# Plachtaa/FAcodec

Measured on AMD Instinct MI355X. Metric: 24kHz audio sec encoded+decoded per wall-sec, higher is better.
Workload: dtype f32; 1 GPU; configs[1]: batch=32/GPU x 2 s @ 24 kHz, forward encoder->FVQ(6 codebooks)->decoder, FAcodec configs/config.yml model (137.7 M params), weights formula-generated, weight-norm re-materialised every step; clips_per_gpu=32, samples_per_clip=48000, parallelism=dp1 (independent clips, no collective)

## Files before the change

### facodec_amd/_lib.py

```python
import ctypes as C
import os

_HERE = os.path.dirname(os.path.abspath(__file__))
LIB_PATH = os.environ.get("FAC_LIB_PATH", os.path.join(_HERE, "libfacodec_hip.so"))

PAD_ZERO, PAD_REFLECT = 0, 1
ACT_NONE, ACT_TANH, ACT_MISH, ACT_LOG_MEL = 0, 1, 2, 3
ACT_GATE, ACT_WN_RES_SKIP = 4, 5

_p = C.c_void_p
_i = C.c_int
_i64 = C.c_int64
_f = C.c_float


class ConvDesc(C.Structure):
    _fields_ = [
        ("x", _p), ("w", _p), ("bias", _p), ("alpha_in", _p), ("alpha_out", _p), ("res", _p), ("y", _p), ("y2", _p), ("alpha_y2", _p), ("w_k1", _p), ("bias_k1", _p),
        ("x_bs", _i64), ("x_cs", _i64), ("y_bs", _i64), ("y_cs", _i64),
        ("B", C.c_int32), ("C_in", C.c_int32), ("T_in", C.c_int32), ("C_out", C.c_int32),
        ("C_out_pad", C.c_int32), ("T_out", C.c_int32),
        ("K", C.c_int32), ("stride", C.c_int32), ("dilation", C.c_int32), ("pad_left", C.c_int32),
        ("pad_mode", C.c_int32), ("n_phase", C.c_int32), ("y_tstride", C.c_int32), ("phase_shift", C.c_int32),
        ("act", C.c_int32),
        ("w_batched", C.c_int32), ("w_bs", _i64), ("ws", _p), ("ws_bytes", _i64), ("w_split", _p),
        ("K1", C.c_int32), ("dilation2", C.c_int32), ("row_phases", C.c_int32),
        ("x_p8", _p), ("x_p8_plane_bytes", _i64), ("y2_p8", _p), ("y2_p8_plane_bytes", _i64),
        ("pw_split", C.c_int32), ("split_rows", C.c_int32),
        ("gate_cond", _p), ("gate_cond_bs", _i64),
    ]


class VqDesc(C.Structure):
    _fields_ = [
        ("residual", _p), ("z_in", _p), ("zq_acc", _p), ("zq_out", _p), ("w_in", _p), ("b_in", _p),
        ("codebook", _p), ("w_out", _p), ("w_out_scale", _p), ("b_out", _p), ("mask", _p), ("codes", _p), ("z_e", _p),
        ("loss_part", _p), ("codes_bs", _i64),
        ("B", C.c_int32), ("D", C.c_int32), ("T", C.c_int32), ("Kc", C.c_int32),
    ]



VQ_DECODE_MAX_Q = 16


class VqDecodeDesc(C.Structure):
    _fields_ = [
        ("codes", _p * 3), ("codes_bs", _i64 * 3), ("codes_qs", _i64 * 3), ("n_q", C.c_int32 * 3),
        ("codebook", _p * VQ_DECODE_MAX_Q), ("w_out", _p * VQ_DECODE_MAX_Q), ("w_out_scale", _p * VQ_DECODE_MAX_Q),
        ("b_out", _p * VQ_DECODE_MAX_Q), ("style", _p), ("outs", _p), ("z", _p * 3),
        ("B", C.c_int32), ("D", C.c_int32), ("T", C.c_int32), ("Kc", C.c_int32),
    ]


class CodesPackDesc(C.Structure):
    _fields_ = [
        ("codes", _p * 3), ("codes_bs", _i64 * 3), ("codes_qs", _i64 * 3), ("n_q", C.c_int32 * 3),
        ("lens", _p), ("out", _p), ("out_bs", _i64),
        ("B", C.c_int32), ("T", C.c_int32), ("bits", C.c_int32),
    ]


# ... 147 lines not shown
    "fac_spec_to_cat": (_i, [_p, _p, _i, _i, _i, _i, _i, _i, _i, _p]),
    "fac_period_fold": (_i, [_p, _p, _i, _i, _i, _i, _i, _i, _p]),
    "fac_zero_insert": (_i, [_p, _p, _i64, _i, _i, _p]),
    "fac_row_stack3": (_i, [_p, _p, _i64, _i, _i, _i, _i, _p]),
    "fac_spec_to_rows": (_i, [_p, _p, _i, _i, _i, _i, _i, _i, _p]),
    "fac_pad_reflect": (_i, [_p, _p, _i, _i, _i, _i, _p]),
    "fac_disc_preprocess": (_i, [_p, _p, _p, _p, _i, _i, _p]),
    "fac_cross_entropy": (_i, [_p, _p, _p, _p, _p, _i64, _i, _f, _p]),
    "fac_focal_scalar": (_i, [_p, _p, _f, _p]),
    "fac_crop_rows": (_i, [_p, _p, _p, _i, _i, _i64, _i, _i, _p]),
    "fac_stream_push": (_i, [_p, _p, _i64, _i64, _i, _i, _i, _p]),
    "fac_vq_fwd": (_i, [C.POINTER(VqDesc), _p]),
    "fac_vq_loss_tiles": (_i, [_i]),
    "fac_vq_decode": (_i, [C.POINTER(VqDecodeDesc), _p]),
    "fac_codes_pack": (_i, [C.POINTER(CodesPackDesc), _p]),
    "fac_codes_unpack": (_i, [C.POINTER(CodesUnpackDesc), _p]),
    "fac_codes_row_bytes": (_i64, [_i, _i, _i]),
    "fac_rccl_available": (_i, []),
    "fac_rccl_unique_id": (_i, [_p]),
    "fac_rccl_comm_init": (_i, [C.POINTER(_p), _p, _i, _i]),
    "fac_rccl_comm_destroy": (_i, [_p]),
    "fac_allreduce_arena": (_i, [_p, _p, _i64, _i, _p]),
    "fac_vq_search": (_i, [_p, _p, _p, _i64, _i, _p]),
    "fac_gate_tanh_sigmoid": (_i, [_p, _p, _i64, _p, _i, _i, _i, _p]),
    "fac_embed_sum": (_i, [_p, _p, _p, _i, _i, _i, _i, _i, _i, _i, _i, _p]),
    "fac_glu_residual": (_i, [_p, _p, _p, _i, _i, _i, _p]),
    "fac_add": (_i, [_p, _p, _p, _i64, _p]),
    "fac_sub2": (_i, [_p, _p, _p, _p, _i64, _p]),
    "fac_mul_mask": (_i, [_p, _p, _i, _i, _i, _p]),
    "fac_wn_res_skip": (_i, [_p, _p, _p, _i, _i, _i, _i, _p]),
    "fac_attention": (_i, [_p, _p, _p, _p, _p, _i, _i, _i, _i, _p]),
    "fac_attention_stream": (_i, [_p, _p, _p, _p, _p, _i, _i, _i, _i, _p]),
    "fac_attention_route": (_i, [_i, _i]),
    "fac_attention_stream_tile": (_i, [_i]),
    "fac_masked_mean": (_i, [_p, _p, _p, _i, _i, _i, _p]),
    "fac_layernorm_c_affine": (_i, [_p, _p, _p, _i, _i, _i, _p]),
    "fac_stft_frames": (_i, [_p, _p, _i, _i, _i, _i, _i, _i, _i, _p]),
    "fac_stft_frames_ragged": (_i, [_p, _p, _p, _i, _i, _i, _i, _i, _i, _i, _p]),
    "fac_mask_tail": (_i, [_p, _p, _i, _i, _i, _i, _p]),
    "fac_mask_tail_i64": (_i, [_p, _p, _i, _i, _i, _i, _p]),
    "fac_edge_tail": (_i, [_p, _p, _i, _i, _i, _i, _i, _i, _p]),
    "fac_frame_mask": (_i, [_p, _p, _p, _i, _i, _i, _p]),
    "fac_resample": (_i, [C.POINTER(ResampleDesc), _p]),
    "fac_resample_form": (_i, [C.POINTER(ResampleDesc), _p]),
    "fac_kweight_ws_bytes": (_i64, [_i, _i]),
    "fac_kweight_energy": (_i, [C.POINTER(KweightDesc), _p]),
    "fac_loudness_chunk": (_i, [_i]),
    "fac_loudness_gate": (_i, [_p, _i64, _p, _i64, _i, _i, _p, _i, _p, _p, _i, _p]),
    "fac_loudness_gain": (_i, [_p, _i64, _p, _p, _p, _p, C.c_double, _i, _p, _i64, _p, _i, _i, _p]),
    "fac_si_sdr_ws_bytes": (_i64, [_i, _i]),
    "fac_si_sdr": (_i, [_p, _i64, _p, _i64, _p, _p, _p, _i64, _i, _i, _p]),
    "fac_stoi_geometry": (_i, [_i, C.POINTER(_i64)]),
    "fac_stoi_select": (_i, [C.POINTER(StoiDesc), _p]),
    "fac_stoi_bands": (_i, [C.POINTER(StoiDesc), _p]),
    "fac_stoi_score": (_i, [C.POINTER(StoiDesc), _p]),
    "fac_slot_copy": (_i, [_p, _i, _p, _i, _i, _i, C.POINTER(C.c_int32), _i, _p]),
    "fac_rows_pick": (_i, [_p, _i64, _p, _p, _i, _i, _i, _p]),
    "fac_spec_power": (_i, [_p, _p, _i, _i, _i, _i, _p]),
    "fac_reduce_pair": (_i, [_p, _p, _p, _p, _i64, _i, _f, _f, _i, _p]),
    "fac_aa_snakebeta_fwd": (_i, [_p, _p, _p, _p, _p, _i, _i, _i, _p]),
    "fac_logdiff_rms": (_i, [_p, _p, _p, _p, _i, _i, _i, _f, _f, _i, _p]),
    "fac_jdc_affine_lrelu_pool": (_i, [_p, _p, _p, _p, _i, _i, _i, _i, _i, _i, _i, _f, _p]),
    "fac_jdc_layout_in": (_i, [_p, _p, _i, _i, _i, _i, _p]),
    "fac_jdc_to_time_major": (_i, [_p, _p, _i, _i, _i, _i, _i, _i, _i, _p]),
    "fac_jdc_to_nchw": (_i, [_p, _p, _i, _i, _i, _i, _i, _i, _p]),
    "fac_jdc_head": (_i, [_p, _p, _p, _p, _p, _i, _i, _i, _i, _p]),
# ... 34 lines not shown
```

### facodec_amd/build.py

```python
import os
import subprocess
import sys
from concurrent.futures import ThreadPoolExecutor

HERE = os.path.dirname(os.path.abspath(__file__))
CSRC = os.path.join(HERE, "csrc")
TAG = os.environ.get("FAC_BUILD_TAG", "")
LIB = os.path.join(HERE, "libfacodec_hip%s.so" % ("_" + TAG if TAG else ""))
OBJDIR = "build" + ("_" + TAG if TAG else "")
SOURCES = ["conv1d_api.hip", "conv1d_tile_128x128.hip", "conv1d_tile_96x128.hip", "conv1d_tile_64x128.hip",
           "conv1d_tile_32x256.hip", "conv1d_tile_128x32.hip", "conv1d_tile_128x256.hip", "conv1d_fused_ru.hip", "conv1d_narrow.hip", "conv1d_pw.hip", "conv1d_pw_split.hip", "conv1d_skinny.hip", "conv1d_bsplit.hip", "conv1d_bsplit96.hip", "conv1d_gemm_split.hip", "conv1d_bsplit2.hip", "conv1d_bwd.hip", "conv1d_wgrad_split.hip", "conv1d_wgrad_k1.hip", "train_misc.hip", "optim.hip", "train_quant.hip", "train_pred.hip", "train_disc.hip", "train_redecoder.hip", "pack.hip", "prep_batch.hip", "lstm.hip", "lstm_persist.hip", "vq.hip", "vq_decode.hip", "bitpack.hip", "misc.hip", "attention_stream.hip", "ragged.hip", "resample.hip", "loudness.hip", "metrics.hip", "stream_pool.hip", "jdc.hip", "rccl_arena.hip"]
FLAGS = ["--offload-arch=gfx950", "-O3", "-std=c++17", "-fPIC", "-ffp-contract=off",
         "-Wno-unused-result"] + os.environ.get("FAC_EXTRA_FLAGS", "").split()


def _hipcc():
    for cand in (os.environ.get("HIPCC"), "/opt/rocm/bin/hipcc", "hipcc"):
        if cand and (os.path.isabs(cand) and os.path.exists(cand) or not os.path.isabs(cand)):
            return cand
    return "hipcc"


def _stale(target, deps):
    if not os.path.exists(target):
        return True
    tt = os.path.getmtime(target)
    return any(os.path.getmtime(d) > tt for d in deps)


def build_lib(force=False, verbose=True):
    hipcc = _hipcc()
    headers = sorted(os.path.join(CSRC, f) for f in os.listdir(CSRC) if f.endswith(".h")) + [os.path.join(HERE, "..", "include", "facodec_hip.h")]
    objs, jobs = [], []
    os.makedirs(os.path.join(CSRC, OBJDIR), exist_ok=True)
    for src in SOURCES:
        s = os.path.join(CSRC, src)
        o = os.path.join(CSRC, OBJDIR, src.replace(".hip", ".o"))
        objs.append(o)
        if force or _stale(o, [s] + headers):
            jobs.append([hipcc, *FLAGS, "-c", s, "-o", o])

    def run(cmd):
        if verbose:
            print(" ".join(cmd), file=sys.stderr)
# ... 13 lines not shown
```

### facodec_amd/csrc/conv1d_api.hip

```cpp
#include "conv1d_mfma.h"
#include <stdlib.h>

namespace fac {

enum ConvKernel : int {
  CK_128x32 = 0,
  CK_32x256 = 1,
  CK_64x128 = 2,
  CK_96x128 = 3,
  CK_128x128 = 4,
  CK_128x256 = 5,
  CK_96x256 = 6,
  CK_FUSED_RU = 7,
  CK_128x160 = 8,
  CK_NARROW = 9,
  CK_SKINNY = 10,
  CK_BSPLIT = 11,
  CK_CIN1 = 12,
  CK_THIN = 13,
  CK_PW = 14,
  CK_GSPLIT = 15,
  CK_BSPLIT2 = 16,
  CK_PWS = 17,
  CK_PWT = 18,
  CK_BSPLIT96 = 19,
};

static ConvKernel select_variant(const fac_conv_desc* d) {
  const int co = d->C_out;
  if (d->row_phases > 1) return CK_128x256;
  if (d->T_out <= 32) return CK_128x32;
  if (co <= 32) return CK_32x256;
  if (co <= 64) return CK_64x128;
  const bool wide = d->K == 1 && d->n_phase == 1 && d->T_out >= 512;
  if (d->T_out > 128 && d->T_out <= 160 && co > 64) return CK_128x160;
  if (co % 128 != 0 && co % 96 == 0) return wide ? CK_96x256 : CK_96x128;
  return wide ? CK_128x256 : CK_128x128;
}

static bool narrow_ok(const fac_conv_desc* d) {
  return d->C_out <= 2 && d->stride == 1 && d->n_phase == 1 && d->phase_shift == 0 && d->y_tstride == 1 && !d->res && !d->y2 &&
         !d->w_batched && d->y && (long long)d->B <= 65535 && (long long)d->B * ((d->T_out + 1023) / 1024) >= 128;
}

static bool pw_enabled() {
  static const bool on = !(getenv("FAC_PW") && getenv("FAC_PW")[0] == '0');
  return on;
}

static int conv_plan(const fac_conv_desc* d, ConvArgs& a, ConvKernel& k) {
  FAC_REQUIRE(d && (d->x || d->x_p8) && (d->w || d->w_split) && (d->y || d->y2 || d->y2_p8), "conv1d: null pointer");
  FAC_REQUIRE(!d->y2 || d->alpha_y2 || d->act == FAC_ACT_WN_RES_SKIP, "conv1d: y2 needs alpha_y2");
  FAC_REQUIRE(d->B > 0 && d->C_in > 0 && d->C_out > 0 && d->T_in > 0 && d->T_out > 0,
              "conv1d: bad shape B=%d C_in=%d C_out=%d T_in=%d T_out=%d", d->B, d->C_in, d->C_out,
              d->T_in, d->T_out);
  FAC_REQUIRE(d->K >= 1 && d->stride >= 1 && d->dilation >= 1 && d->pad_left >= 0,
              "conv1d: bad K/stride/dilation/pad");
  FAC_REQUIRE(d->C_out_pad % 32 == 0 && (d->C_out_pad >= d->C_out || d->row_phases > 1), "conv1d: C_out_pad must be a multiple of 32");
  FAC_REQUIRE(d->n_phase >= 1 && d->y_tstride >= 1, "conv1d: bad phase config");
  FAC_REQUIRE((long long)d->B * d->n_phase <= 65535, "conv1d: B*n_phase too large for grid.z");
  a.x = d->x; a.w = d->w; a.bias = d->bias; a.alpha_in = d->alpha_in; a.alpha_out = d->alpha_out;
  a.res = d->res; a.y = d->y; a.y2 = d->y2; a.alpha2 = d->alpha_y2;
  a.w1 = d->w_k1; a.bias1 = d->bias_k1;
  a.x_p8 = reinterpret_cast<const unsigned char*>(d->x_p8); a.x_p8_ps = d->x_p8_plane_bytes;
  a.y2_p8 = reinterpret_cast<unsigned char*>(d->y2_p8); a.y2_p8_ps = d->y2_p8_plane_bytes;
  FAC_REQUIRE(!d->y2_p8 || d->alpha_y2, "conv1d: y2_p8 needs alpha_y2");
  if (d->w_k1) {
    FAC_REQUIRE(d->C_in == d->C_out && d->C_out_pad == d->C_out && d->n_phase == 1 && d->stride == 1 &&
// ... 168 lines not shown
```

### facodec_amd/csrc/misc.hip

```cpp
#include "common.h"
#include <string.h>

namespace fac {

static thread_local char g_err[512] = "";

void set_error(const char* fmt, ...) {
  va_list ap;
  va_start(ap, fmt);
  vsnprintf(g_err, sizeof(g_err), fmt, ap);
  va_end(ap);
}

constexpr int EW_THREADS = 256;
inline int ew_grid(long long n, int per_thread = 1) {
  long long g = (n + (long long)EW_THREADS * per_thread - 1) / ((long long)EW_THREADS * per_thread);
  if (g > 8192) g = 8192;
  if (g < 1) g = 1;
  return (int)g;
}

__global__ void snake_kernel(const float* __restrict__ x, const float* __restrict__ alpha,
                             float* __restrict__ y, int C, int T, long long n) {
  for (long long i = (long long)blockIdx.x * blockDim.x + threadIdx.x; i < n;
// ... 537 lines not shown
  if (threadIdx.x == 0) scratch[blockIdx.x] = (part[0] + part[1]) + (part[2] + part[3]);
}

__global__ __launch_bounds__(256) void logdiff_rms_bwd_kernel(const float* __restrict__ a, const float* __restrict__ b,
                                                              float* __restrict__ db, int M, int T, long long n_cols, float eps,
                                                              float scale, int accumulate) {
  for (long long i = (long long)blockIdx.x * 256 + threadIdx.x; i < n_cols; i += (long long)gridDim.x * 256) {
    const long long bb = i / T;
    const int t = (int)(i - bb * T);
    const float* pa = a + bb * M * T + t;
    const float* pb = b + bb * M * T + t;
    float* pd = db + bb * M * T + t;
    float q = 0.f;
    for (int m = 0; m < M; ++m) {
      const float d = logf(fabsf(pa[(long long)m * T]) + eps) - logf(fabsf(pb[(long long)m * T]) + eps);
      q = fmaf(d, d, q);
    }
    const float r = sqrtf(q / (float)M);
    const float k = r > 0.f ? scale / ((float)M * r) : 0.f;
    for (int m = 0; m < M; ++m) {
      const float bv = pb[(long long)m * T];
      const float d = logf(fabsf(pa[(long long)m * T]) + eps) - logf(fabsf(bv) + eps);
      const float sg = bv > 0.f ? 1.f : (bv < 0.f ? -1.f : 0.f);
      const float g = -k * d * sg / (fabsf(bv) + eps);
      pd[(long long)m * T] = accumulate ? pd[(long long)m * T] + g : g;
    }
  }
}

}

using namespace fac;

extern "C" int fac_version(void) { return 4; }
extern "C" const char* fac_last_error(void) { return fac::g_err; }

#define EW_LAUNCH(kern, n, ...)                                                         \
  hipLaunchKernelGGL(kern, dim3(ew_grid(n)), dim3(EW_THREADS), 0, (hipStream_t)stream, __VA_ARGS__)

extern "C" int fac_snake_fwd(const float* x, const float* alpha, float* y, int B, int C, int T,
                             fac_stream_t stream) {
  FAC_REQUIRE(x && alpha && y && B > 0 && C > 0 && T > 0, "snake_fwd: bad arguments");
  const long long n = (long long)B * C * T;
  if (T >= 1024 && (long long)B * C <= 65535) {
    hipLaunchKernelGGL(snake_rows_kernel, dim3((T + 1023) / 1024, B * C), dim3(256), 0, (hipStream_t)stream, x, alpha, y, C, T);
  } else {
    EW_LAUNCH(snake_kernel, n, x, alpha, y, C, T, n);
  }
  return check_launch("snake_fwd");
}

extern "C" int fac_gate_tanh_sigmoid(const float* a, const float* g, int64_t g_bs, float* out, int B,
                                     int C, int T, fac_stream_t stream) {
  FAC_REQUIRE(a && out && B > 0 && C > 0 && T > 0, "gate_tanh_sigmoid: bad arguments");
  const long long n = (long long)B * C * T;
  EW_LAUNCH(gate_kernel, n, a, g, out, C, T, (long long)g_bs, n);
  return check_launch("gate_tanh_sigmoid");
}

extern "C" int fac_embed_sum(const int64_t* codes, const float* tables, float* out, int B, int n_tab,
                             int n_codes, int code_row0, int V, int E, int T, int accumulate,
                             fac_stream_t stream) {
  FAC_REQUIRE(codes && tables && out && B > 0 && n_tab >= 0 && V > 0 && E > 0 && T > 0 &&
                  code_row0 >= 0 && code_row0 + n_tab <= n_codes, "embed_sum: bad arguments");
  const long long n = (long long)B * E * T;
  EW_LAUNCH(embed_sum_kernel, n, (const long long*)codes, tables, out, n_tab, n_codes, code_row0, V, E, T, n,
            accumulate);
// ... 21 lines not shown
  return check_launch("sub2");
}

extern "C" int fac_mul_mask(float* x, const float* mask, int B, int C, int T, fac_stream_t stream) {
  FAC_REQUIRE(x && mask && B > 0 && C > 0 && T > 0, "mul_mask: bad arguments");
  const long long n = (long long)B * C * T;
  EW_LAUNCH(mul_mask_kernel, n, x, mask, C, T, n);
  return check_launch("mul_mask");
}

extern "C" int fac_stream_push(float* buf, const float* src, int64_t rows, int64_t cap, int hist, int n_prev,
                               int n_new, fac_stream_t stream) {
  FAC_REQUIRE(buf && src && rows > 0 && hist >= 0 && hist <= 2048 && n_prev >= 0 && n_new > 0 &&
                  cap >= (int64_t)hist + n_new && cap >= (int64_t)hist + n_prev,
              "stream_push: bad arguments (rows=%lld cap=%lld hist=%d n_prev=%d n_new=%d)", (long long)rows,
              (long long)cap, hist, n_prev, n_new);
  hipLaunchKernelGGL(stream_push_kernel, dim3((unsigned)rows), dim3(256), 0, (hipStream_t)stream, buf, src,
                     (long long)cap, hist, n_prev, n_new);
  return check_launch("stream_push");
}

extern "C" int fac_wn_res_skip(const float* rs, float* x, float* out, int B, int C, int T, int last,
                               fac_stream_t stream) {
  FAC_REQUIRE(rs && out && (last || x) && B > 0 && C > 0 && T > 0, "wn_res_skip: bad arguments");
  const long long n = (long long)B * C * T;
  EW_LAUNCH(wn_res_skip_kernel, n, rs, x, out, C, T, last, n);
  return check_launch("wn_res_skip");
}

extern "C" int fac_attention_route(int dk, int T) {
  return ((size_t)dk * 16 + (size_t)16 * T) * sizeof(float) <= FAC_LDS_MAX ? FAC_ATTN_LDS : FAC_ATTN_STREAM;
}

extern "C" int fac_attention(const float* q, const float* k, const float* v, const float* mask,
                             float* out, int B, int n_heads, int dk, int T, fac_stream_t stream) {
  FAC_REQUIRE(q && k && v && out && B > 0 && n_heads > 0 && dk > 0 && T > 0, "attention: bad arguments");
  if (fac_attention_route(dk, T) == FAC_ATTN_STREAM) return fac_attention_stream(q, k, v, mask, out, B, n_heads, dk, T, stream);
  size_t lds = ((size_t)dk * 16 + (size_t)16 * T) * sizeof(float);
  const size_t lds_v = lds + (size_t)16 * (T + 1) * sizeof(float);
  const int stage_v = lds_v <= FAC_LDS_MAX ? 1 : 0;
  if (stage_v) lds = lds_v;
  allow_dynamic_lds<attention_kernel>();
  dim3 grid((T + 15) / 16, n_heads, B);
  hipLaunchKernelGGL(attention_kernel, grid, dim3(256), lds, (hipStream_t)stream, q, k, v, mask, out,
                     n_heads, dk, T, stage_v);
  return check_launch("attention");
}

extern "C" int fac_masked_mean(const float* x, const float* mask, float* out, int B, int C, int T,
                               fac_stream_t stream) {
  FAC_REQUIRE(x && out && B > 0 && C > 0 && T > 0, "masked_mean: bad arguments");
  hipLaunchKernelGGL(masked_mean_kernel, dim3(C, B), dim3(64), 0, (hipStream_t)stream, x, mask, out, C, T);
  return check_launch("masked_mean");
}

extern "C" int fac_layernorm_c_affine(const float* x, const float* style, float* out, int B, int C,
                                      int T, fac_stream_t stream) {
  FAC_REQUIRE(x && style && out && B > 0 && C > 0 && T > 0, "layernorm_c_affine: bad arguments");
  if (T <= 8 && (size_t)C * T * 4 <= 64 * 1024) {
    hipLaunchKernelGGL(layernorm_c_small_t_kernel, dim3(B), dim3(256), (size_t)C * T * 4, (hipStream_t)stream, x,
                       style, out, C, T);
    return check_launch("layernorm_c_affine(small T)");
  }
  hipLaunchKernelGGL(layernorm_c_kernel, dim3((T + 63) / 64, B), dim3(256), 0, (hipStream_t)stream, x,
                     style, out, C, T);
  return check_launch("layernorm_c_affine");
}

extern "C" int fac_stft_frames(const float* wave, float* frames, int B, int T, int n_win,
                               int n_frames, int hop, int pad, int n_off, fac_stream_t stream) {
// ... 131 lines not shown
```

### facodec_amd/ops.py

```python
import ctypes as C
import math
import os
from collections import namedtuple

import torch

from . import _lib
from .wprep import prepared
from .convplan import *
from ._lib import ConvDesc, VqDesc, VqDecodeDesc, ResampleDesc, PAD_REFLECT, PAD_ZERO, ACT_NONE, ACT_TANH, ACT_MISH, ACT_LOG_MEL, ACT_GATE, ACT_WN_RES_SKIP


def pad32(n):
    return (n + 31) & ~31


def cin_pad(c):
    return ((c + 47) // 48) * 48


_RAW_STREAM = getattr(torch._C, "_cuda_getCurrentRawStream", None)
_GET_DEVICE = getattr(torch._C, "_cuda_getDevice", None)


# ... 415 lines not shown


P8_PREPASS_MIN_FLOP_PER_BYTE = 450.0


def p8_prepass(x, flop_per_in_byte):
    if (flop_per_in_byte is None or P8_PREPASS_MIN_FLOP_PER_BYTE <= 0 or flop_per_in_byte < P8_PREPASS_MIN_FLOP_PER_BYTE or not BF16_SPLIT or isinstance(x, P8)
            or torch.is_grad_enabled() or not x.is_cuda or x.shape[1] % 8 != 0 or x.shape[0] * (x.shape[1] // 8) * x.shape[2] * 16 >= (1 << 32)):
        return x
    return to_p8(x)


def conv_y_channels(c_out, act):
    return c_out // 2 if act in (ACT_GATE, ACT_WN_RES_SKIP) else c_out


def conv_desc(B, c_in, t_in, c_out, k, stride=1, dilation=1, pad_left=None, pad_mode=PAD_REFLECT, t_out=None, act=ACT_NONE, causal=True,
              k1=0, dilation2=0, c_out_pad=None, split_rows=0):
    if pad_left is None:
        t_o, padding_total, _ = conv_out_len(t_in, k, stride, dilation)
        pad_left = padding_total if causal else padding_total - padding_total // 2
        if t_out is None:
            t_out = t_o
    if t_out is None:
        raise ValueError("t_out required with explicit pad_left")
    d = ConvDesc()
    d.x_bs, d.x_cs = c_in * t_in, t_in
    d.y_bs, d.y_cs = conv_y_channels(c_out, act) * t_out, t_out
    d.B, d.C_in, d.T_in, d.C_out, d.C_out_pad, d.T_out = B, c_in, t_in, c_out, (pad32(c_out) if c_out_pad is None else c_out_pad), t_out
    d.K, d.stride, d.dilation, d.pad_left, d.pad_mode = k, stride, dilation, pad_left, pad_mode
    d.n_phase, d.y_tstride, d.act, d.w_batched, d.w_bs = 1, 1, act, 0, 0
    d.K1, d.dilation2, d.split_rows = k1, dilation2, split_rows
    d.pw_split = 1 if (BF16_SPLIT and PW_SPLIT and (k == 1 or (PW_TAPS and k == 4 and stride == 2))) else 0
    return d


def conv1d(x, w_packed, c_out, k, bias=None, stride=1, dilation=1, pad_left=None, pad_mode=PAD_REFLECT,
           t_out=None, alpha_in=None, alpha_out=None, res=None, act=ACT_NONE, out=None, causal=True,
           alpha_y2=None, want_y=True, w_k1=None, bias_k1=None, w_split=None, k1=0, dilation2=0, skip_acc=None, gate_cond=None):
    x_p8 = x if isinstance(x, P8) else None
    if x_p8 is not None:
        B, c_in, t_in = x_p8.shape
    else:
        if not (x.is_cuda and x.dtype == torch.float32 and x.dim() == 3 and x.stride(2) == 1):
            x = _dev(x, "x")
        B, c_in, t_in = x.shape
    dev_ = x_p8.planes.device if x_p8 is not None else x.device
    d = conv_desc(B, c_in, t_in, c_out, k, stride, dilation, pad_left, pad_mode, t_out, act, causal, k1, dilation2,
                  w_packed.shape[-1] if w_packed is not None else None,
                  getattr(w_split, "split_rows", 0))
    t_out, c_y = d.T_out, conv_y_channels(c_out, act)
    if out is None and want_y:
        out = torch.empty(B, c_y, t_out, device=dev_, dtype=torch.float32)
    y2 = torch.empty(B, c_out, t_out, device=dev_, dtype=torch.float32) if alpha_y2 is not None else None
    if act == ACT_WN_RES_SKIP:
        assert skip_acc is not None and skip_acc.is_contiguous() and skip_acc.shape == out.shape and alpha_y2 is None
        y2 = skip_acc
    res = _dev(res, "res")
    d.bias = bias.data_ptr() if bias is not None else None
    if x_p8 is not None:
        d.x, d.x_p8, d.x_p8_plane_bytes = None, x_p8.planes.data_ptr(), x_p8.plane_bytes
    else:
        d.x = x.data_ptr()
        d.x_bs, d.x_cs = x.stride(0), x.stride(1)
    d.w = w_packed.data_ptr() if w_packed is not None else w_split.data_ptr()
    d.alpha_in = alpha_in.data_ptr() if alpha_in is not None else None
# ... 50 lines not shown
        if not (has_history and x.is_cuda and x.dtype == torch.float32 and x.stride(2) == 1):
            x = _dev(x, "x")
        B, c_in, t_in = x.shape
    dev_ = x_p8.planes.device if x_p8 is not None else x.device
    if has_history:
        assert causal
    split_rows = isinstance(w_packed, tuple)
    d = convtr_desc(B, c_in, t_in, c_out, stride, w_packed[1] if split_rows else w_packed.shape[-1], causal, has_history,
                    not split_rows and w_packed.dim() == 3, split_rows)
    if out is None:
        out = torch.empty(B, c_out, d.T_out * stride, device=dev_, dtype=torch.float32)
    d.bias = bias.data_ptr() if bias is not None else None
    if x_p8 is not None:
        d.x, d.x_p8, d.x_p8_plane_bytes = None, x_p8.planes.data_ptr(), x_p8.plane_bytes
    else:
        d.x = x.data_ptr()
        d.x_bs, d.x_cs = x.stride(0), x.stride(1)
    if split_rows:
        d.w, d.w_split = None, w_packed[0].data_ptr()
    else:
        d.w = w_packed.data_ptr()
    d.alpha_in = alpha_in.data_ptr() if alpha_in is not None else None
    d.alpha_out, d.res, d.y = None, None, out.data_ptr()
    y2 = torch.empty_like(out) if alpha_y2 is not None else None
    d.y2 = y2.data_ptr() if y2 is not None else None
    d.alpha_y2 = alpha_y2.data_ptr() if alpha_y2 is not None else None
    _launch_conv(d, "fac_conv1d_fwd(convtr)")
    return (out, y2) if alpha_y2 is not None else out


FLAT_TRAIN = True
PW_SPLIT = os.environ.get("FAC_PW_SPLIT", "1") != "0"
PW_TAPS = True


def pack_conv_for(layout, v, g, stride=1, k1=0, scale=None):
    if layout in (W_FP32, W_FP32_PW_TAPS):
        return pack_conv_weight(v, g, scale=scale), None
    if layout == W_GEMM_STRIDED:
        return None, pack_gemm_weight_split(v, g, in_stride=stride, scale=scale)
    if layout == W_SPLIT2:
        return None, pack_conv_weight_split2(v, g, k1, scale=scale)
    return None, pack_conv_weight_split(v, g, scale=scale, rows=64)


def pack_convtr_for(layout, v, g, stride):
    if layout in (TR_ROWS_SPLIT, TR_FLAT):
        return pack_convtr_weight_rows_split(v, g, stride)
    return pack_convtr_weight(v, g, stride) if layout == TR_POLYPHASE else pack_convtr_weight_rows(v, g, stride)


def convtr_weight_for(v, g, stride, t_in, causal=True, batch=1, alpha_in=None):
    return pack_convtr_for(plan_convtr(v.shape[0], v.shape[1], stride, batch, t_in, causal=causal, alpha_in=alpha_in is not None).layout,
                           v, g, stride)


def flat_conv_cols(B, L, s, n):
    pitch = L // s
    return pitch, B * L, B * pitch - (pitch - n)


def flat_convtr_cols(B, T1):
    return B * T1


def conv1d_flat(xp, w_split, c_out, k, s, n, dilation=1, bias=None, p8=None, alpha_out=None, act=ACT_NONE, alpha_y2=None, want_y=True):
# ... 435 lines not shown
    _lib.check(_lib.load().fac_add(_ptr(a), _ptr(b), _ptr(out), a.numel(), _stream()), "fac_add")
    return out


def sub2(a, b, c, out=None):
    a, b, c = _dev(a), _dev(b), _dev(c)
    if out is None:
        out = torch.empty_like(a)
    _lib.check(_lib.load().fac_sub2(_ptr(a), _ptr(b), _ptr(c), _ptr(out), a.numel(), _stream()), "fac_sub2")
    return out


def mul_mask_(x, mask):
    B, c, T = x.shape
    _lib.check(_lib.load().fac_mul_mask(_ptr(x), _ptr(mask), B, c, T, _stream()), "fac_mul_mask")
    return x


def wn_res_skip_(rs, x, out, last):
    B, c, T = out.shape
    _lib.check(_lib.load().fac_wn_res_skip(_ptr(rs), _ptr(x), _ptr(out), B, c, T, 1 if last else 0, _stream()),
               "fac_wn_res_skip")


def attention_route(dk, T):
    return ("lds", "stream")[_lib.load().fac_attention_route(int(dk), int(T))]


def attention_stream_tiles():
    lib = _lib.load()
    return lib.fac_attention_stream_tile(0), lib.fac_attention_stream_tile(1)


def attention(q, k, v, mask, n_heads, kernel=None):
    if kernel not in (None, "lds", "stream"):
        raise ValueError(f"attention: kernel={kernel!r} (None, 'lds' or 'stream')")
    q, k, v = _dev(q), _dev(k), _dev(v)
    B, c, T = q.shape
    dk = c // n_heads
    out = torch.empty_like(q)
    if kernel == "lds" and attention_route(dk, T) != "lds":
        raise _lib.FacodecHipError(f"attention: T={T} too long for the LDS score tile at dk={dk}")
    name = "fac_attention_stream" if kernel == "stream" else "fac_attention"
    _lib.check(getattr(_lib.load(), name)(_ptr(q), _ptr(k), _ptr(v), _ptr(mask), _ptr(out), B, n_heads, dk, T, _stream()), name)
    return out


def masked_mean(x, mask):
    x = _dev(x)
    B, c, T = x.shape
    out = torch.empty(B, c, device=x.device, dtype=torch.float32)
    _lib.check(_lib.load().fac_masked_mean(_ptr(x), _ptr(mask), _ptr(out), B, c, T, _stream()), "fac_masked_mean")
    return out


def layernorm_c_affine(x, style):
    x, style = _dev(x), _dev(style)
    B, c, T = x.shape
    out = torch.empty_like(x)
    _lib.check(_lib.load().fac_layernorm_c_affine(_ptr(x), _ptr(style), _ptr(out), B, c, T, _stream()),
               "fac_layernorm_c_affine")
    return out


def stft_frames(wave, n_win, n_frames, hop, pad, n_off):
    wave = _dev(wave, "wave")
    B, T = wave.shape
    frames = torch.empty(B, n_win, n_frames, device=wave.device, dtype=torch.float32)
    _lib.check(_lib.load().fac_stft_frames(_ptr(wave), _ptr(frames), B, T, n_win, n_frames, hop, pad, n_off, _stream()),
               "fac_stft_frames")
    return frames


def _lens(lens, B):
    if not isinstance(lens, torch.Tensor) or not lens.is_cuda:
        raise _lib.FacodecHipError(f"lens must live on the GPU (got {getattr(lens, 'device', type(lens))}); there is no CPU path")
# ... 915 lines not shown
```

### include/facodec_hip.h

```cpp
#ifndef FACODEC_HIP_H
#define FACODEC_HIP_H

#include <stdint.h>

#ifdef __cplusplus
extern "C" {
#endif

typedef void* fac_stream_t;

#define FAC_OK 0
#define FAC_ERR_ARG (-1)
#define FAC_ERR_LAUNCH (-2)

#define FAC_PAD_ZERO 0
#define FAC_PAD_REFLECT 1

#define FAC_ACT_NONE 0
#define FAC_ACT_TANH 1
#define FAC_ACT_MISH 2
#define FAC_ACT_LOG_MEL 3
#define FAC_ACT_GATE 4
#define FAC_ACT_WN_RES_SKIP 5

// ... 25 lines not shown
  const float* bias;
  const float* alpha_in;
  const float* alpha_out;
  const float* res;
  float* y;
  float* y2;
  const float* alpha_y2;
  const float* w_k1;
  const float* bias_k1;
  int64_t x_bs, x_cs;
  int64_t y_bs, y_cs;
  int32_t B, C_in, T_in, C_out, C_out_pad;
  int32_t T_out;
  int32_t K, stride, dilation, pad_left, pad_mode;
  int32_t n_phase;
  int32_t y_tstride;
  int32_t phase_shift;
  int32_t act;
  int32_t w_batched;
  int64_t w_bs;
  void* ws;
  int64_t ws_bytes;
  const void* w_split;
  int32_t K1, dilation2;
  int32_t row_phases;
  const void* x_p8;
  int64_t x_p8_plane_bytes;
  void* y2_p8;
  int64_t y2_p8_plane_bytes;
  int32_t pw_split;
  int32_t split_rows;
  const float* gate_cond;
  int64_t gate_cond_bs;
} fac_conv_desc;

int fac_conv1d_fwd(const fac_conv_desc* d, fac_stream_t stream);
int fac_to_p8(const float* x, const float* alpha, void* out, int B, int C, int T, fac_stream_t stream);
int64_t fac_conv_w_split_bytes(int C_out, int C_in, int K);
int64_t fac_conv_w_split_rows_bytes(int C_out, int C_in, int K, int rows);
int fac_pack_conv_w_split_rows(const float* v, const float* scale, void* out, int C_out, int C_in, int K, int rows, fac_stream_t stream);
int fac_pack_conv_w_split(const float* v, const float* scale, void* out, int C_out, int C_in, int K,
                          fac_stream_t stream);
int64_t fac_conv_w_split2_bytes(int C_out, int C_in, int K, int K1);
int fac_pack_conv_w_split2(const float* v, const float* scale, void* out, int C_out, int C_in, int K, int K1, fac_stream_t stream);
int64_t fac_gemm_w_split_bytes(int R, int C_in, int K, int in_stride);
int fac_pack_gemm_w_split(const float* v, int64_t row_stride, int64_t ci_stride, int64_t k_stride, const float* row_scale, void* out,
                          int R, int C_in, int K, int in_stride, fac_stream_t stream);
int fac_conv1d_variant(const fac_conv_desc* d, char* name, int name_len);

int fac_snake_fwd(const float* x, const float* alpha, float* y, int B, int C, int T,
                  fac_stream_t stream);


int fac_lstm_to_time_major(const float* x, float* xT, int B, int H, int T, fac_stream_t stream);
int fac_lstm_from_time_major(const float* yT, const float* skip, const float* alpha, float* out, int B, int H, int T,
                             fac_stream_t stream);
int fac_pack_lstm_whh(const float* w_hh, float* packed, int H, fac_stream_t stream);
int fac_lstm_layer_fwd(const float* pre, const float* whh_packed, float* yT, float* c, int T,
                       int H, int BP, fac_stream_t stream);
int fac_lstm_layer_fwd_from(const float* pre, const float* whh_packed, float* yT, float* c, int T,
                            int H, int BP, int64_t step0, fac_stream_t stream);
int fac_lstm_layer_fwd_train(const float* pre, const float* whh_packed, float* yT, float* c, float* gates_save,
                             float* c_save, int T, int H, int BP, int64_t step0, fac_stream_t stream);
int fac_lstm_gate_bwd(const float* dy_t, const float* rec, const float* gates_t, const float* c_t, const float* c_prev,
                      float* dc, float* dgates_t, int H, int BP, int64_t rs, int first, fac_stream_t stream);
int fac_pack_lstm_whh_t(const float* w_hh, float* packed, int H, fac_stream_t stream);
// ... 183 lines not shown
  int64_t codes_qs[3];
  int32_t n_q[3];
  const int32_t* lens;
  int32_t B, T, bits;
} fac_codes_unpack_desc;

int fac_codes_pack(const fac_codes_pack_desc* d, fac_stream_t stream);
int fac_codes_unpack(const fac_codes_unpack_desc* d, fac_stream_t stream);
int64_t fac_codes_row_bytes(int T, int Q, int bits);

int fac_vq_search(const float* latents, const float* codebook, int64_t* idx, int64_t N, int Kc,
                  fac_stream_t stream);


int fac_gate_tanh_sigmoid(const float* a, const float* g, int64_t g_bs, float* out, int B, int C, int T,
                          fac_stream_t stream);
int fac_embed_sum(const int64_t* codes, const float* tables, float* out, int B, int n_tab, int n_codes,
                  int code_row0, int V, int E, int T, int accumulate, fac_stream_t stream);
int fac_glu_residual(const float* a, const float* res, float* out, int B, int C, int T,
                     fac_stream_t stream);
int fac_add(const float* a, const float* b, float* out, int64_t n, fac_stream_t stream);
int fac_sub2(const float* a, const float* b, const float* c, float* out, int64_t n,
             fac_stream_t stream);
int fac_mul_mask(float* x, const float* mask, int B, int C, int T, fac_stream_t stream);
int fac_wn_res_skip(const float* rs, float* x, float* out, int B, int C, int T, int last,
                    fac_stream_t stream);
int fac_attention(const float* q, const float* k, const float* v, const float* mask, float* out,
                  int B, int n_heads, int dk, int T, fac_stream_t stream);
int fac_attention_stream(const float* q, const float* k, const float* v, const float* mask, float* out,
                         int B, int n_heads, int dk, int T, fac_stream_t stream);
#define FAC_ATTN_LDS 0
#define FAC_ATTN_STREAM 1
int fac_attention_route(int dk, int T);
int fac_attention_stream_tile(int which);
int fac_masked_mean(const float* x, const float* mask, float* out, int B, int C, int T,
                    fac_stream_t stream);
int fac_layernorm_c_affine(const float* x, const float* style, float* out, int B, int C, int T,
                           fac_stream_t stream);


int fac_stft_frames(const float* wave, float* frames, int B, int T, int n_win, int n_frames,
                    int hop, int pad, int n_off, fac_stream_t stream);


int fac_stft_frames_ragged(const float* wave, const int32_t* lens, float* frames, int B, int T, int n_win, int n_frames,
                           int hop, int pad, int n_off, fac_stream_t stream);
int fac_mask_tail(float* x, const int32_t* lens, int B, int C, int T, int unit, fac_stream_t stream);
int fac_mask_tail_i64(int64_t* x, const int32_t* lens, int B, int C, int T, int unit, fac_stream_t stream);
int fac_edge_tail(float* x, const int32_t* lens, int B, int C, int T, int mul, int n, int mode, fac_stream_t stream);
int fac_frame_mask(const int32_t* lens, float* mask, int32_t* n_valid, int B, int F, int unit, fac_stream_t stream);
int fac_spec_power(const float* spec, float* out, int B, int F, int n_frames, int power,
                   fac_stream_t stream);
int fac_reduce_pair(const float* a, const float* b, float* out, float* scratch, int64_t n,
                    int mode, float eps, float scale, int accumulate, fac_stream_t stream);

int fac_aa_snakebeta_fwd(const float* x, const float* alpha_log, const float* beta_log,
                         const float* filter12, float* y, int B, int C, int T, fac_stream_t stream);

int fac_logdiff_rms(const float* a, const float* b, float* out, float* scratch, int B, int M, int T,
                    float eps, float scale, int accumulate, fac_stream_t stream);

int fac_logdiff_rms_bwd(const float* a, const float* b, float* db, int B, int M, int T, float eps, float scale,
                        int accumulate, fac_stream_t stream);

typedef struct fac_resample_desc {
  const float* hist;
// ... 96 lines not shown
```

Baseline: 1255 audio-s/s.

## Add tiled attention kernel and route short K=1 convs to 128x32 tiles

Adds a new attention kernel that processes 32 query columns per block, with Q staged in LDS and a full score row, then a softmax and a V pass through LDS. Compared with the older 16-query serial kernel it is meant to reuse K/V loads across more queries. The default attention route now uses it whenever it fits. Separately, pointwise convs with T_out in 129..160 and few output-channel tiles now use the 128x32 tile instead of 128x160 to get more blocks. Risks are higher register/LDS pressure and lower occupancy in the new attention kernel.

```diff
diff --git a/facodec_amd/_lib.py b/facodec_amd/_lib.py
--- a/facodec_amd/_lib.py
+++ b/facodec_amd/_lib.py
@@ -28,6 +28,7 @@
         ("x_p8", _p), ("x_p8_plane_bytes", _i64), ("y2_p8", _p), ("y2_p8_plane_bytes", _i64),
         ("pw_split", C.c_int32), ("split_rows", C.c_int32),
         ("gate_cond", _p), ("gate_cond_bs", _i64),
+        ("keep_tile160", C.c_int32),
     ]
 
 
@@ -241,6 +242,10 @@
     "fac_attention": (_i, [_p, _p, _p, _p, _p, _i, _i, _i, _i, _p]),
     "fac_attention_stream": (_i, [_p, _p, _p, _p, _p, _i, _i, _i, _i, _p]),
     "fac_attention_route": (_i, [_i, _i]),
+    "fac_attention_form": (_i, [_i, _i]),
+    "fac_attention_tiled_fits": (_i, [_i, _i]),
+    "fac_attention_tiled": (_i, [_p, _p, _p, _p, _p, _i, _i, _i, _i, _p]),
+    "fac_attention_serial": (_i, [_p, _p, _p, _p, _p, _i, _i, _i, _i, _p]),
     "fac_attention_stream_tile": (_i, [_i]),
     "fac_masked_mean": (_i, [_p, _p, _p, _i, _i, _i, _p]),
     "fac_layernorm_c_affine": (_i, [_p, _p, _p, _i, _i, _i, _p]),
diff --git a/facodec_amd/build.py b/facodec_amd/build.py
--- a/facodec_amd/build.py
+++ b/facodec_amd/build.py
@@ -9,7 +9,7 @@
 LIB = os.path.join(HERE, "libfacodec_hip%s.so" % ("_" + TAG if TAG else ""))
 OBJDIR = "build" + ("_" + TAG if TAG else "")
 SOURCES = ["conv1d_api.hip", "conv1d_tile_128x128.hip", "conv1d_tile_96x128.hip", "conv1d_tile_64x128.hip",
-           "conv1d_tile_32x256.hip", "conv1d_tile_128x32.hip", "conv1d_tile_128x256.hip", "conv1d_fused_ru.hip", "conv1d_narrow.hip", "conv1d_pw.hip", "conv1d_pw_split.hip", "conv1d_skinny.hip", "conv1d_bsplit.hip", "conv1d_bsplit96.hip", "conv1d_gemm_split.hip", "conv1d_bsplit2.hip", "conv1d_bwd.hip", "conv1d_wgrad_split.hip", "conv1d_wgrad_k1.hip", "train_misc.hip", "optim.hip", "train_quant.hip", "train_pred.hip", "train_disc.hip", "train_redecoder.hip", "pack.hip", "prep_batch.hip", "lstm.hip", "lstm_persist.hip", "vq.hip", "vq_decode.hip", "bitpack.hip", "misc.hip", "attention_stream.hip", "ragged.hip", "resample.hip", "loudness.hip", "metrics.hip", "stream_pool.hip", "jdc.hip", "rccl_arena.hip"]
+           "conv1d_tile_32x256.hip", "conv1d_tile_128x32.hip", "conv1d_tile_128x256.hip", "conv1d_fused_ru.hip", "conv1d_narrow.hip", "conv1d_pw.hip", "conv1d_pw_split.hip", "conv1d_skinny.hip", "conv1d_bsplit.hip", "conv1d_bsplit96.hip", "conv1d_gemm_split.hip", "conv1d_bsplit2.hip", "conv1d_bwd.hip", "conv1d_wgrad_split.hip", "conv1d_wgrad_k1.hip", "train_misc.hip", "optim.hip", "train_quant.hip", "train_pred.hip", "train_disc.hip", "train_redecoder.hip", "pack.hip", "prep_batch.hip", "lstm.hip", "lstm_persist.hip", "vq.hip", "vq_decode.hip", "bitpack.hip", "misc.hip", "attention_stream.hip", "attention_tiled.hip","ragged.hip", "resample.hip", "loudness.hip", "metrics.hip", "stream_pool.hip", "jdc.hip", "rccl_arena.hip"]
 FLAGS = ["--offload-arch=gfx950", "-O3", "-std=c++17", "-fPIC", "-ffp-contract=off",
          "-Wno-unused-result"] + os.environ.get("FAC_EXTRA_FLAGS", "").split()
 
diff --git a/facodec_amd/csrc/attention_tiled.hip b/facodec_amd/csrc/attention_tiled.hip
--- /dev/null
+++ b/facodec_amd/csrc/attention_tiled.hip
@@ -0,0 +1,205 @@
+#include "common.h"
+
+namespace fac {
+
+constexpr int ATTN_TILED_QT = 32;
+constexpr int ATTN_TILED_KC = 32;
+constexpr int ATTN_TILED_VS = ATTN_TILED_KC + 4;
+constexpr int ATTN_TILED_DK = 256;
+static_assert(ATTN_TILED_DK * ATTN_TILED_QT <= ATTN_TILED_DK * ATTN_TILED_VS, "the queries share the V pass's LDS");
+
+static inline int attn_tiled_ts(int T) { return (T + ATTN_TILED_KC - 1) / ATTN_TILED_KC * ATTN_TILED_KC; }
+static inline size_t attn_tiled_lds(int T) {
+  return ((size_t)ATTN_TILED_DK * ATTN_TILED_VS + (size_t)ATTN_TILED_QT * attn_tiled_ts(T)) * sizeof(float);
+}
+
+__device__ __forceinline__ float4 attn_ld4(const float* __restrict__ row, int t, int T, bool vec, float fill) {
+  if (vec) return t < T ? *reinterpret_cast<const float4*>(row + t) : make_float4(fill, fill, fill, fill);
+  float4 r;
+  r.x = t < T ? row[t] : fill;
+  r.y = t + 1 < T ? row[t + 1] : fill;
+  r.z = t + 2 < T ? row[t + 2] : fill;
+  r.w = t + 3 < T ? row[t + 3] : fill;
+  return r;
+}
+
+__device__ __forceinline__ float attn_f4(const float4& v, int i) { return i == 0 ? v.x : i == 1 ? v.y : i == 2 ? v.z : v.w; }
+
+__global__ __launch_bounds__(256) void attention_tiled_kernel(const float* __restrict__ q, const float* __restrict__ k,
+                                                              const float* __restrict__ v, const float* __restrict__ mask,
+                                                              float* __restrict__ out, int n_heads, int dk, int T, int TS, int vec) {
+  constexpr int QT = ATTN_TILED_QT, KC = ATTN_TILED_KC, VS = ATTN_TILED_VS;
+  extern __shared__ __align__(16) float sm[];
+  float* qs = sm;
+  float* vs = sm;
+  float* sc = sm + ATTN_TILED_DK * VS;
+  const int lane = threadIdx.x & 63, wave = threadIdx.x >> 6;
+  const int tq0 = blockIdx.x * QT, j0 = wave * 8;
+  const int h = blockIdx.y, b = blockIdx.z;
+  const long long base = ((long long)b * n_heads + h) * dk * T;
+  const float* qg = q + base;
+  const float* kg = k + base;
+  const float* vg = v + base;
+  const float* mrow = mask ? mask + (long long)b * T : nullptr;
+  const float scale = sqrtf((float)dk);
+  for (int i = threadIdx.x; i < dk * QT; i += 256) {
+    const int d = i / QT, j = i - d * QT;
+    const int tq = tq0 + j;
+    qs[i] = tq < T ? __fdiv_rn(qg[(long long)d * T + tq], scale) : 0.f;
+  }
+  __syncthreads();
+
+  float mq[8];
+#pragma unroll
+  for (int jj = 0; jj < 8; ++jj) mq[jj] = mrow && tq0 + j0 + jj < T ? mrow[tq0 + j0 + jj] : 1.f;
+  for (int kb = 0; kb < TS; kb += 256) {
+    const int tk0 = kb + lane * 4;
+    float4 acc[8];
+#pragma unroll
+    for (int jj = 0; jj < 8; ++jj) acc[jj] = make_float4(0.f, 0.f, 0.f, 0.f);
+    float4 cur[8], nxt[8];
+#pragma unroll
+    for (int u = 0; u < 8; ++u) cur[u] = u < dk ? attn_ld4(kg + (long long)u * T, tk0, T, vec, 0.f) : make_float4(0.f, 0.f, 0.f, 0.f);
+    for (int d0 = 0; d0 < dk; d0 += 8) {
+#pragma unroll
+      for (int u = 0; u < 8; ++u) {
+        const int dn = d0 + 8 + u;
+        nxt[u] = dn < dk ? attn_ld4(kg + (long long)dn * T, tk0, T, vec, 0.f) : make_float4(0.f, 0.f, 0.f, 0.f);
+      }
+#pragma unroll
+      for (int u = 0; u < 8; ++u) {
+        if (d0 + u < dk) {
+          const float4 qa = *reinterpret_cast<const float4*>(qs + (d0 + u) * QT + j0);
+          const float4 qb = *reinterpret_cast<const float4*>(qs + (d0 + u) * QT + j0 + 4);
+#pragma unroll
+          for (int jj = 0; jj < 8; ++jj) {
+            const float qv = jj < 4 ? attn_f4(qa, jj) : attn_f4(qb, jj - 4);
+            acc[jj].x = fmaf(qv, cur[u].x, acc[jj].x);
+            acc[jj].y = fmaf(qv, cur[u].y, acc[jj].y);
+            acc[jj].z = fmaf(qv, cur[u].z, acc[jj].z);
+            acc[jj].w = fmaf(qv, cur[u].w, acc[jj].w);
+          }
+        }
+      }
+#pragma unroll
+      for (int u = 0; u < 8; ++u) cur[u] = nxt[u];
+    }
+    if (tk0 < TS) {
+      float mk[4];
+#pragma unroll
+      for (int i = 0; i < 4; ++i) mk[i] = mrow && tk0 + i < T ? mrow[tk0 + i] : 1.f;
+#pragma unroll
+      for (int jj = 0; jj < 8; ++jj) {
+        const bool live = mrow && tq0 + j0 + jj < T;
+        float s[4] = {acc[jj].x, acc[jj].y, acc[jj].z, acc[jj].w};
+#pragma unroll
+        for (int i = 0; i < 4; ++i) {
+          if (live && mq[jj] * mk[i] == 0.f) s[i] = -1e4f;
+          if (tk0 + i >= T) s[i] = 0.f;
+        }
+        *reinterpret_cast<float4*>(sc + (j0 + jj) * TS + tk0) = make_float4(s[0], s[1], s[2], s[3]);
+      }
+    }
+  }
+
+  float4 pf[8];
+  const int srow = threadIdx.x >> 3, scol = (threadIdx.x & 7) * 4;
+#pragma unroll
+  for (int u = 0; u < 8; ++u) {
+    const int r = srow + 32 * u;
+    pf[u] = r < dk ? attn_ld4(vg + (long long)r * T, scol, T, vec, -0.f) : make_float4(0.f, 0.f, 0.f, 0.f);
+  }
+  __syncthreads();
+
+  for (int j = wave; j < QT && tq0 + j < T; j += 4) {
+    float mx = -INFINITY;
+    for (int tk = lane; tk < T; tk += 64) mx = fmaxf(mx, sc[j * TS + tk]);
+#pragma unroll
+    for (int o = 32; o > 0; o >>= 1) mx = fmaxf(mx, __shfl_xor(mx, o, 64));
+    float sum = 0.f;
+    for (int tk = lane; tk < T; tk += 64) {
+      const float e = expf(sc[j * TS + tk] - mx);
+      sc[j * TS + tk] = e;
+      sum += e;
+    }
+#pragma unroll
+    for (int o = 32; o > 0; o >>= 1) sum += __shfl_xor(sum, o, 64);
+    for (int tk = lane; tk < T; tk += 64) sc[j * TS + tk] = __fdiv_rn(sc[j * TS + tk], sum);
+  }
+  __syncthreads();
+
+  float acc[4][8];
+#pragma unroll
+  for (int dd = 0; dd < 4; ++dd)
+#pragma unroll
+    for (int jj = 0; jj < 8; ++jj) acc[dd][jj] = 0.f;
+  for (int tk0 = 0; tk0 < TS; tk0 += KC) {
+    if (tk0) __syncthreads();
+#pragma unroll
+    for (int u = 0; u < 8; ++u) *reinterpret_cast<float4*>(vs + (srow + 32 * u) * VS + scol) = pf[u];
+    __syncthreads();
+    if (tk0 + KC < TS) {
+#pragma unroll
+      for (int u = 0; u < 8; ++u) {
+        const int r = srow + 32 * u;
+        pf[u] = r < dk ? attn_ld4(vg + (long long)r * T, tk0 + KC + scol, T, vec, -0.f) : make_float4(0.f, 0.f, 0.f, 0.f);
+      }
+    }
+#pragma unroll
+    for (int t4 = 0; t4 < KC; t4 += 4) {
+      float4 pp[8], vv[4];
+#pragma unroll
+      for (int jj = 0; jj < 8; ++jj) pp[jj] = *reinterpret_cast<const float4*>(sc + (j0 + jj) * TS + tk0 + t4);
+#pragma unroll
+      for (int dd = 0; dd < 4; ++dd)
+        if (dd * 64 < dk) vv[dd] = *reinterpret_cast<const float4*>(vs + (lane + 64 * dd) * VS + t4);
+#pragma unroll
+      for (int i = 0; i < 4; ++i)
+#pragma unroll
+        for (int dd = 0; dd < 4; ++dd)
+          if (dd * 64 < dk) {
+#pragma unroll
+            for (int jj = 0; jj < 8; ++jj) acc[dd][jj] = fmaf(attn_f4(pp[jj], i), attn_f4(vv[dd], i), acc[dd][jj]);
+          }
+    }
+  }
+#pragma unroll
+  for (int dd = 0; dd < 4; ++dd) {
+    const int d = lane + 64 * dd;
+    if (d < dk) {
+      float* orow = out + base + (long long)d * T + tq0 + j0;
+#pragma unroll
+      for (int g = 0; g < 8; g += 4) {
+        if (vec) {
+          if (tq0 + j0 + g < T) *reinterpret_cast<float4*>(orow + g) = make_float4(acc[dd][g], acc[dd][g + 1], acc[dd][g + 2], acc[dd][g + 3]);
+        } else {
+#pragma unroll
+          for (int jj = g; jj < g + 4; ++jj)
+            if (tq0 + j0 + jj < T) orow[jj] = acc[dd][jj];
+        }
+      }
+    }
+  }
+}
+
+}
+
+using namespace fac;
+
+extern "C" int fac_attention_tiled_fits(int dk, int T) {
+  return dk > 0 && T > 0 && dk <= ATTN_TILED_DK && T <= (1 << 20) && attn_tiled_lds(T) <= FAC_LDS_MAX ? 1 : 0;
+}
+
+extern "C" int fac_attention_tiled(const float* q, const float* k, const float* v, const float* mask, float* out, int B,
+                                   int n_heads, int dk, int T, fac_stream_t stream) {
+  FAC_REQUIRE(q && k && v && out && B > 0 && n_heads > 0 && dk > 0 && T > 0, "attention_tiled: bad arguments");
+  FAC_REQUIRE(fac_attention_tiled_fits(dk, T), "attention_tiled: dk=%d T=%d outside the tiled layout (dk <= %d, T <= 992)", dk, T,
+              ATTN_TILED_DK);
+  FAC_REQUIRE(B <= 65535 && n_heads <= 65535, "attention_tiled: B or heads above 65535");
+  const int vec = T % 4 == 0 && ((uintptr_t)q | (uintptr_t)k | (uintptr_t)v | (uintptr_t)out) % 16 == 0;
+  allow_dynamic_lds<attention_tiled_kernel>();
+  dim3 grid((T + ATTN_TILED_QT - 1) / ATTN_TILED_QT, n_heads, B);
+  hipLaunchKernelGGL(attention_tiled_kernel, grid, dim3(256), attn_tiled_lds(T), (hipStream_t)stream, q, k, v, mask, out, n_heads,
+                     dk, T, attn_tiled_ts(T), vec);
+  return check_launch("attention_tiled");
+}
diff --git a/facodec_amd/csrc/conv1d_api.hip b/facodec_amd/csrc/conv1d_api.hip
--- a/facodec_amd/csrc/conv1d_api.hip
+++ b/facodec_amd/csrc/conv1d_api.hip
@@ -33,7 +33,11 @@
   if (co <= 32) return CK_32x256;
   if (co <= 64) return CK_64x128;
   const bool wide = d->K == 1 && d->n_phase == 1 && d->T_out >= 512;
-  if (d->T_out > 128 && d->T_out <= 160 && co > 64) return CK_128x160;
+  if (d->T_out > 128 && d->T_out <= 160 && co > 64) {
+    const long long wide_tiles = (long long)d->B * ((co + 127) / 128);
+    if (d->K == 1 && d->stride == 1 && d->n_phase == 1 && !d->keep_tile160 && wide_tiles < 256) return CK_128x32;
+    return CK_128x160;
+  }
   if (co % 128 != 0 && co % 96 == 0) return wide ? CK_96x256 : CK_96x128;
   return wide ? CK_128x256 : CK_128x128;
 }
diff --git a/facodec_amd/csrc/misc.hip b/facodec_amd/csrc/misc.hip
--- a/facodec_amd/csrc/misc.hip
+++ b/facodec_amd/csrc/misc.hip
@@ -593,7 +593,7 @@
 
 using namespace fac;
 
-extern "C" int fac_version(void) { return 4; }
+extern "C" int fac_version(void) { return 5; }
 extern "C" const char* fac_last_error(void) { return fac::g_err; }
 
 #define EW_LAUNCH(kern, n, ...)                                                         \
@@ -681,10 +681,23 @@
   return ((size_t)dk * 16 + (size_t)16 * T) * sizeof(float) <= FAC_LDS_MAX ? FAC_ATTN_LDS : FAC_ATTN_STREAM;
 }
 
+extern "C" int fac_attention_form(int dk, int T) {
+  if (fac_attention_route(dk, T) == FAC_ATTN_STREAM) return FAC_ATTN_FORM_STREAM;
+  return fac_attention_tiled_fits(dk, T) ? FAC_ATTN_FORM_TILED : FAC_ATTN_FORM_SERIAL;
+}
+
 extern "C" int fac_attention(const float* q, const float* k, const float* v, const float* mask,
                              float* out, int B, int n_heads, int dk, int T, fac_stream_t stream) {
   FAC_REQUIRE(q && k && v && out && B > 0 && n_heads > 0 && dk > 0 && T > 0, "attention: bad arguments");
   if (fac_attention_route(dk, T) == FAC_ATTN_STREAM) return fac_attention_stream(q, k, v, mask, out, B, n_heads, dk, T, stream);
+  if (fac_attention_form(dk, T) == FAC_ATTN_FORM_TILED) return fac_attention_tiled(q, k, v, mask, out, B, n_heads, dk, T, stream);
+  return fac_attention_serial(q, k, v, mask, out, B, n_heads, dk, T, stream);
+}
+
+extern "C" int fac_attention_serial(const float* q, const float* k, const float* v, const float* mask,
+                                    float* out, int B, int n_heads, int dk, int T, fac_stream_t stream) {
+  FAC_REQUIRE(q && k && v && out && B > 0 && n_heads > 0 && dk > 0 && T > 0, "attention_serial: bad arguments");
+  FAC_REQUIRE(fac_attention_route(dk, T) == FAC_ATTN_LDS, "attention_serial: T=%d too long for the LDS score tile at dk=%d", T, dk);
   size_t lds = ((size_t)dk * 16 + (size_t)16 * T) * sizeof(float);
   const size_t lds_v = lds + (size_t)16 * (T + 1) * sizeof(float);
   const int stage_v = lds_v <= FAC_LDS_MAX ? 1 : 0;
diff --git a/facodec_amd/ops.py b/facodec_amd/ops.py
--- a/facodec_amd/ops.py
+++ b/facodec_amd/ops.py
@@ -471,6 +471,7 @@
     d.n_phase, d.y_tstride, d.act, d.w_batched, d.w_bs = 1, 1, act, 0, 0
     d.K1, d.dilation2, d.split_rows = k1, dilation2, split_rows
     d.pw_split = 1 if (BF16_SPLIT and PW_SPLIT and (k == 1 or (PW_TAPS and k == 4 and stride == 2))) else 0
+    d.keep_tile160 = 0 if K1_COLUMN_TILES else 1
     return d
 
 
@@ -587,6 +588,7 @@
 FLAT_TRAIN = True
 PW_SPLIT = os.environ.get("FAC_PW_SPLIT", "1") != "0"
 PW_TAPS = True
+K1_COLUMN_TILES = True
 
 
 def pack_conv_for(layout, v, g, stride=1, k1=0, scale=None):
@@ -1088,16 +1090,20 @@
     return lib.fac_attention_stream_tile(0), lib.fac_attention_stream_tile(1)
 
 
+def attention_form(dk, T):
+    return ("tiled", "serial", "stream")[_lib.load().fac_attention_form(int(dk), int(T))]
+
+
 def attention(q, k, v, mask, n_heads, kernel=None):
-    if kernel not in (None, "lds", "stream"):
-        raise ValueError(f"attention: kernel={kernel!r} (None, 'lds' or 'stream')")
+    if kernel not in (None, "lds", "stream", "serial"):
+        raise ValueError(f"attention: kernel={kernel!r} (None, 'lds', 'stream' or 'serial')")
     q, k, v = _dev(q), _dev(k), _dev(v)
     B, c, T = q.shape
     dk = c // n_heads
     out = torch.empty_like(q)
-    if kernel == "lds" and attention_route(dk, T) != "lds":
+    if kernel in ("lds", "serial") and attention_route(dk, T) != "lds":
         raise _lib.FacodecHipError(f"attention: T={T} too long for the LDS score tile at dk={dk}")
-    name = "fac_attention_stream" if kernel == "stream" else "fac_attention"
+    name = {"stream": "fac_attention_stream", "serial": "fac_attention_serial"}.get(kernel, "fac_attention")
     _lib.check(getattr(_lib.load(), name)(_ptr(q), _ptr(k), _ptr(v), _ptr(mask), _ptr(out), B, n_heads, dk, T, _stream()), name)
     return out
 
diff --git a/include/facodec_hip.h b/include/facodec_hip.h
--- a/include/facodec_hip.h
+++ b/include/facodec_hip.h
@@ -81,6 +81,7 @@
   int32_t split_rows;
   const float* gate_cond;
   int64_t gate_cond_bs;
+  int32_t keep_tile160;
 } fac_conv_desc;
 
 int fac_conv1d_fwd(const fac_conv_desc* d, fac_stream_t stream);
@@ -330,6 +331,15 @@
 #define FAC_ATTN_LDS 0
 #define FAC_ATTN_STREAM 1
 int fac_attention_route(int dk, int T);
+#define FAC_ATTN_FORM_TILED 0
+#define FAC_ATTN_FORM_SERIAL 1
+#define FAC_ATTN_FORM_STREAM 2
+int fac_attention_form(int dk, int T);
+int fac_attention_tiled_fits(int dk, int T);
+int fac_attention_tiled(const float* q, const float* k, const float* v, const float* mask, float* out,
+                        int B, int n_heads, int dk, int T, fac_stream_t stream);
+int fac_attention_serial(const float* q, const float* k, const float* v, const float* mask, float* out,
+                         int B, int n_heads, int dk, int T, fac_stream_t stream);
 int fac_attention_stream_tile(int which);
 int fac_masked_mean(const float* x, const float* mask, float* out, int B, int C, int T,
                     fac_stream_t stream);
```

Measured after the change: 1270 audio-s/s, median of 6. +1.2%, better.
